# mountaindust/Parasitoids

Hardware: AMD Instinct MI355X
Metric: grid-days/sec on 4096^2 fp64 domain (higher is better)
Workload: dtype f64; 1 GPU; C3 synthetic stack: N=4097 (nominal 4096^2), 30 Gaussian day kernels K=2049, reference torus P=5121, FFT size 5184 (fast mode), prob model, one replica stack per GPU; dom_len=4097, ndays=30, P=5121, fft_len=5184, kernels_direct=False, full_column_pipeline=True

## Files before the change

parasitoids_amd/csrc/fft_colfull_kernels.h:

```cpp
#pragma once
#include "fft_rs_kernels.h"

struct ColFullArgs {
  const cplx* src;
  int64_t src_bstride;
  cplx* state;
  int64_t state_bstride;
  cplx* dst;
  int64_t dst_bstride;
  int ld, ncols, mode, store_prod;
  int nd;
  int dst_t;
  int dst_jb, dst_cc, dst_rst;
  int64_t src_dstride, dst_dstride;
  RowLive live;
  const unsigned long long* pred;
  double* pad_energy;
  int pad_row0, ncols_total;
  int col0;
  const cplx* alt_src;
  const unsigned long long* alt_pred;
  RowLive alt_live;
  FftProg prog;
};
// ... 263 lines not shown
#pragma unroll
          for (int q = 0; q < R1; ++q) x[q] = sst[jv + q * S::T1];
        }
        if (day + 1 < nd) fetch(day + 1, jv);
      }
      if constexpr (MODE == 0 && !CHAIN) {
        __syncthreads();
        if (jv < S::T3) {
#pragma unroll
          for (int q = 0; q < R3; ++q) ex[jv + q * S::T3] = x[q].x;
        }
        __syncthreads();
        if (jv < S::T1) {
#pragma unroll
          for (int q = 0; q < R1; ++q) x[q].x = ex[jv + q * S::T1];
        }
        __syncthreads();
        if (jv < S::T3) {
#pragma unroll
          for (int q = 0; q < R3; ++q) ex[jv + q * S::T3] = x[q].y;
        }
        __syncthreads();
        if (jv < S::T1) {
#pragma unroll
          for (int q = 0; q < R1; ++q) x[q].y = ex[jv + q * S::T1];
        }
        __syncthreads();
      }
      if constexpr (MODE == 0) {
        if (CHAIN) asm volatile("" : "+v"(w2.x), "+v"(w2.y), "+v"(w3.x), "+v"(w3.y));
        if (jv < S::T1) bfly<R1, PS_INV>(x);
        rs_tail<S, R1, R2, R3, PS_INV>(x, ex, jv, w2, w3);
        if (jv < S::T3) {
          const int64_t rst = a.dst_rst;
          const unsigned off = PS_COLFULL_OFF(a, c, jv);
          cplx* d = a.dst + (int64_t)blockIdx.y * a.dst_bstride + (int64_t)day * a.dst_dstride;
#pragma unroll
          for (int q = 0; q < R3; ++q) (d + (int64_t)(q * S::T3) * rst)[off] = x[q];
        }
        if (day + 1 < nd) __syncthreads();
      }
    }
    if (chain && a.store_prod && j < S::T3) {
#pragma unroll
      for (int q = 0; q < R3; ++q) st[j + q * S::T3] = sst[j + q * S::T3];
    }
  }
}


static __global__ void k_prefix_cols(cplx* state, cplx* khat, int L, int ncols, int nd) {
  const int k = blockIdx.x * blockDim.x + threadIdx.x;
  if (k >= L) return;
  const int64_t col = (int64_t)blockIdx.y * L + k;
  cplx p = state[col];
  for (int d = 0; d < nd; ++d) {
    cplx* e = khat + ((int64_t)d * ncols) * L + col;
    p = cmul(p, *e);
    *e = p;
  }
  state[col] = p;
}

template <int R1, int R2, int R3>
struct RsDual {
  using S = Rs<R1, R2, R3>;
  static constexpr int L = S::L;
  static constexpr int QA2 = (R2 + 1) / 2, QA3 = (R3 + 1) / 2;
  static constexpr int IA = QA2 * S::T2, IB = QA3 * S::T3;
  static constexpr int JA1 = IA / 16, JA2 = 16 * QA3;
  static constexpr int OFF1 = IA + IA / 16, OFF2 = IB + IB / 16;
  static constexpr int mx(int a, int b) { return a > b ? a : b; }
  static constexpr int MAXEL = mx(mx(IA, L - IA), mx(IB, L - IB));
  static constexpr int XH = (MAXEL + MAXEL / 16 + 32 + 15) & ~15;
  static constexpr size_t fixed_bytes = 2 * (size_t)XH * sizeof(double) + (size_t)L * sizeof(cplx);
  static constexpr long spare = (long)160 * 1024 - (long)fixed_bytes;
  static constexpr int CAP = spare > 0 ? (int)(spare / (64 * (long)sizeof(cplx))) * 64 : 0;
  static constexpr bool ok = S::NTHR <= 384 && CAP >= 512 &&
                             (S::RMAX <= 18 || (S::RMAX == 20 && (R2 * R3 == 20 * 14 || R2 * R3 == 20 * 16)));
  static constexpr size_t bytes = fixed_bytes + (size_t)CAP * sizeof(cplx);
  static_assert(S::T2 % 16 == 0 && S::T3 % 16 == 0, "half-pass offsets assume whole padding groups");
};

template <int R1, int R2, int R3>
__global__ void __launch_bounds__((2 * Rs<R1, R2, R3>::NTHR)) k_colfull_dual(ColFullArgs a) {
  using S = Rs<R1, R2, R3>;
  using D = RsDual<R1, R2, R3>;
  constexpr int L = S::L;
  constexpr int NW = S::NTHR / 64;
  if (pred_skip(a.pred)) return;
  const int b = blockIdx.x, xcd = b & 7, qq = b >> 3;
  const int c = a.col0 + ((((qq >> 3) << 3) + xcd) << 3) + (qq & 7);
  if (c >= a.ncols) return;
  const int role = threadIdx.x / S::NTHR;
  const int j0 = threadIdx.x - role * S::NTHR;
  double* exh = reinterpret_cast<double*>(ps_lds_raw) + role * D::XH;
  cplx* sst = reinterpret_cast<cplx*>(reinterpret_cast<double*>(ps_lds_raw) + 2 * D::XH);
  cplx* stage = sst + L;
  const FftProg& P = a.prog;
  const cplx w2c = tw_lookup(P.tw_lo, P.tw_hi, P.tw_shift, S::tw2(j0));
  const cplx w3c = tw_lookup(P.tw_lo, P.tw_hi, P.tw_shift, j0 < S::T3 ? S::tw3(j0) : 0);
  cplx* st = a.state + (int64_t)blockIdx.y * a.state_bstride + (int64_t)c * L;
  const int nd = a.nd;
  const int lane = j0 & 63, wave = j0 >> 6;

  auto live_of = [&](int day, int& a1, int& b1, int& a2, int& b2) {
    if (!a.live.on) { a1 = 0; b1 = L; a2 = L; b2 = L; return; }
    int lo = 0, hi = 0x3fffffff;
    if (a.live.range) { lo = a.live.range[2 * ((int)blockIdx.y + day)]; hi = a.live.range[2 * ((int)blockIdx.y + day) + 1]; }
    const SrcMap& m = a.live.map;
    a1 = max(0, lo - m.off1); b1 = min(m.n1, hi - m.off1 + 1);
    a2 = m.lo2 + max(0, lo - m.off2); b2 = min(L, m.lo2 + hi - m.off2 + 1);
    if (b1 < a1) b1 = a1;
    if (b2 < a2) b2 = a2;
    if (a2 < b1) a2 = b1;
  };
  auto stage_column = [&](int day) {
    int a1, b1, a2, b2;
    live_of(day, a1, b1, a2, b2);
    const int len1 = b1 - a1, tot = min(len1 + (b2 - a2), D::CAP);
    const cplx* sc = a.src + (int64_t)blockIdx.y * a.src_bstride + (int64_t)day * a.src_dstride + (int64_t)c * L;
    for (int ch = wave; ch * 64 < tot; ch += NW) {
      int e = ch * 64 + lane;
      e = e < tot ? e : tot - 1;
      const int n = e < len1 ? a1 + e : a2 + (e - len1);
      __builtin_amdgcn_global_load_lds(sc + n, (ps_lds_ptr)(stage + ch * 64), 16, 0, 0);
    }
  };

  if (role == 1) {
    stage_column(0);
    PS_WAIT_VM0();
  }
  PS_BAR_LDS();

  for (int slot = 0; slot <= nd; ++slot) {
    const bool act = role == 0 ? slot >= 1 : slot < nd;
    cplx x[S::RMAX];
    int j = j0;
    cplx w2 = w2c, w3 = w3c;
    asm volatile("" : "+v"(j), "+v"(w2.x), "+v"(w2.y), "+v"(w3.x), "+v"(w3.y));
    if (role == 0 && slot == 0) {
#pragma unroll 7
      for (int k = j; k < L; k += S::NTHR) sst[k] = st[k];
    }
    if (act && j < S::T1) {
      if (role == 0) {
#pragma unroll
        for (int q = 0; q < R1; ++q) x[q] = cconj(sst[j + q * S::T1]);
      } else {
        int a1, b1, a2, b2;
        live_of(slot, a1, b1, a2, b2);
        const int len1 = b1 - a1, len2 = b2 - a2;
        if (len1 + len2 <= D::CAP) {
#pragma unroll
          for (int q = 0; q < R1; ++q) {
            const int n = j + q * S::T1;
            const unsigned d1 = (unsigned)(n - a1), d2 = (unsigned)(n - a2);
            const bool in1 = d1 < (unsigned)len1, in2 = d2 < (unsigned)len2;
            const cplx v = stage[in1 ? d1 : (in2 ? len1 + d2 : 0u)];
            x[q] = (in1 || in2) ? v : make_double2(0.0, 0.0);
          }
        } else {
          const cplx* sc = a.src + (int64_t)blockIdx.y * a.src_bstride + (int64_t)slot * a.src_dstride + (int64_t)c * L;
#pragma unroll
          for (int q = 0; q < R1; ++q) {
            const int n = j + q * S::T1;
            x[q] = make_double2(0.0, 0.0);
            int e = -1;
            if (n >= a1 && n < b1) e = n - a1;
            else if (n >= a2 && n < b2) e = len1 + (n - a2);
            if (e >= 0) x[q] = e < D::CAP ? stage[e] : sc[n];
          }
        }
      }
      bfly<R1, PS_FWD>(x);
    }
#pragma unroll
    for (int part = 0; part < 2; ++part) {
      double keep[D::QA2];
#pragma unroll
      for (int h = 0; h < 2; ++h) {
        if (act && j < S::T1 && (j < D::JA1) == (h == 0)) {
          if (part) rs_put<R1, 1>(exh, S::x1_w(j) - h * D::OFF1, 1, x);
          else rs_put<R1, 0>(exh, S::x1_w(j) - h * D::OFF1, 1, x);
        }
        PS_BAR_LDS();
        if (part == 0 && h == 0 && role == 1 && slot + 1 < nd) stage_column(slot + 1);
        if (act && j < S::T2) {
          if (h == 0) {
#pragma unroll
            for (int q = 0; q < D::QA2; ++q) keep[q] = exh[S::x_r(j) + q * S::X1_RS];
          } else {
#pragma unroll
            for (int q = D::QA2; q < R2; ++q) {
              const double v = exh[S::x_r(j) + q * S::X1_RS - D::OFF1];
              if (part) x[q].y = v;
              else x[q].x = v;
            }
#pragma unroll
            for (int q = 0; q < D::QA2; ++q) {
              if (part) x[q].y = keep[q];
              else x[q].x = keep[q];
            }
          }
        }
        if (!(part == 1 && h == 1)) PS_BAR_LDS();
      }
    }
    asm volatile("" : "+v"(w2.x), "+v"(w2.y));
    if (act && j < S::T2) rs_stage<R2, PS_FWD>(x, w2, true);
    PS_BAR_LDS();
#pragma unroll
    for (int part = 0; part < 2; ++part) {
      double keep[D::QA3];
#pragma unroll
      for (int h = 0; h < 2; ++h) {
        if (act && j < S::T2 && (j < D::JA2) == (h == 0)) {
          if (part) rs_put<R2, 1>(exh, S::x2_w(j) - h * D::OFF2, 17, x);
          else rs_put<R2, 0>(exh, S::x2_w(j) - h * D::OFF2, 17, x);
        }
        PS_BAR_LDS();
        if (act && j < S::T3) {
          if (h == 0) {
#pragma unroll
            for (int q = 0; q < D::QA3; ++q) keep[q] = exh[S::x_r(j) + q * S::X2_RS];
          } else {
#pragma unroll
            for (int q = D::QA3; q < R3; ++q) {
              const double v = exh[S::x_r(j) + q * S::X2_RS - D::OFF2];
              if (part) x[q].y = v;
              else x[q].x = v;
            }
#pragma unroll
            for (int q = 0; q < D::QA3; ++q) {
              if (part) x[q].y = keep[q];
              else x[q].x = keep[q];
            }
          }
        }
        if (!(part == 1 && h == 1)) PS_BAR_LDS();
      }
    }
    asm volatile("" : "+v"(w3.x), "+v"(w3.y));
    if (act && j < S::T3) rs_stage<R3, PS_FWD>(x, w3, true);
    if (act && j < S::T3) {
      if (role == 0) {
        const int64_t rst = a.dst_rst;
        cplx* d = a.dst + (int64_t)blockIdx.y * a.dst_bstride + (int64_t)(slot - 1) * a.dst_dstride + PS_COLFULL_OFF(a, c, j);
#pragma unroll
        for (int q = 0; q < R3; ++q) d[(int64_t)(q * S::T3) * rst] = cconj(x[q]);
      } else {
#pragma unroll
        for (int q = 0; q < R3; ++q) {
          const cplx p = cmul(sst[j + q * S::T3], x[q]);
          sst[j + q * S::T3] = p;
        }
      }
    }
    if (role == 1 && slot == nd && a.store_prod) {
      for (int k = j; k < L; k += S::NTHR) st[k] = sst[k];
    }
    if (role == 0 && a.pad_energy) {
      double pe = 0.0;
      if (act && j < S::T3) {
        const int qlo = a.pad_row0 / S::T3;
#pragma unroll
        for (int q = 0; q < R3; ++q) {
          if (q < qlo) continue;
          if (q > qlo || j + q * S::T3 >= a.pad_row0) pe += x[q].x * x[q].x + x[q].y * x[q].y;
        }
      }
      pe = ps_wave_sum(pe);
      if (lane == 63) exh[D::XH - 8 + wave] = pe;
    }
    if (role == 1) PS_WAIT_VM0();
    PS_BAR_LDS();
    if (role == 0 && a.pad_energy && slot >= 1 && j0 == 0) {
      double e = 0.0;
      for (int w = 0; w < NW; ++w) e += exh[D::XH - 8 + w];
      a.pad_energy[((int64_t)blockIdx.y + (slot - 1)) * a.ncols_total + c] = e;
    }
  }
}
```

parasitoids_amd/csrc/ps_coldual.hip:

```cpp
#include "fft_colfull_kernels.h"
#include "rs_cfg.h"
#include "rs_launch.h"

template <int A, int B>
struct DualCfg {
  using D = RsDual<16, A, B>;
  using C = RsCfg<A, B>;
  static constexpr bool on = D::ok && C::CHAIN && C::LDSC > (size_t)80 * 1024;
};

bool rs_dual_ok(int r2, int r3) {
#define X(A, B) \
  if (r2 == A && r3 == B) return DualCfg<A, B>::on;
  PS_RS_SIZES(X)
#undef X
  return false;
}

int rs_coldual_set_attrs() {
#define X(A, B)                                                                                         \
  if constexpr (DualCfg<A, B>::on) {                                                                    \
    using DD = RsDual<16, A, B>;                                                                        \
    auto kern = k_colfull_dual<16, A, B>;                                                               \
    if (hipFuncSetAttribute((const void*)kern, hipFuncAttributeMaxDynamicSharedMemorySize, (int)DD::bytes) != hipSuccess) \
      return -1;                                                                                        \
  }
  PS_RS_SIZES(X)
#undef X
  return 0;
}

int rs_launch_coldual(int r2, int r3, const ColFullArgs& a, int lines8, int batch, hipStream_t st) {
  const dim3 grid((unsigned)(lines8 * 64), batch);
#define X(A, B)                                                                                         \
  if (r2 == A && r3 == B) {                                                                             \
    if constexpr (DualCfg<A, B>::on) {                                                                  \
      using DD = RsDual<16, A, B>;                                                                      \
      auto kern = k_colfull_dual<16, A, B>;                                                             \
      hipLaunchKernelGGL(kern, grid, dim3(2 * DD::S::NTHR), DD::bytes, st, a);                          \
      return 1;                                                                                         \
    }                                                                                                   \
    return 0;                                                                                           \
  }
  PS_RS_SIZES(X)
#undef X
  return 0;
}
```

parasitoids_amd/csrc/ps_config.h:

```cpp
#pragma once
#include <cstdlib>
#include <cstring>

#define PS_OPTION_TABLE(X)                                                                          \
                                               \
  X("PS_NO_RS", no_rs, 0, FLAG, C)                                                                  \
  X("PS_NO_RS_FWD", no_rs_fwd, 0, FLAG, C)                                                          \
  X("PS_NO_BIG_RADIX", no_big_radix, 0, FLAG, C)                                                    \
  X("PS_NO_TPIPE", no_tpipe, 0, FLAG, C)                                                            \
  X("PS_NO_FOLD_TPIPE", no_fold_tpipe, 0, FLAG, C)                                                  \
  X("PS_COL_SINGLE_MAX", col_single_max, 1200, INT, C)                                              \
  X("PS_COL_L1", col_l1, 0, INT, C)                                                                 \
  X("PS_CHUNK_DAYS", chunk_days, 0, INT, C)                                                         \
  X("PS_FAST_SIZE", fast_size, 0, INT, C)                                                           \
  X("PS_RS_AREA", rs_area, 0.0, NUM, C)                                                             \
                                                                                 \
  X("PS_COL_WSH", col_wsh, -1, INT, R)                                                              \
  X("PS_COL_THREADS", col_threads, 256, INT, R)                                                     \
  X("PS_FUSED_WSH", fused_wsh, -1, INT, R)                                                          \
  X("PS_FUSED_THREADS", fused_threads, 0, INT, R)                                                   \
  X("PS_FUSED_G", fused_g, 2, INT, R)                                                               \
  X("PS_MULTI_WSH", multi_wsh, -1, INT, R)                                                          \
  X("PS_DUAL_WSH", dual_wsh, -1, INT, R)                                                            \
  X("PS_FUSED_DAYS", fused_days, 8, INT, R)                                                         \
  X("PS_DIRECT_DAYS", direct_days, 4, INT, R)                                                       \
  X("PS_DIRECT_MAX_TERMS", direct_max_terms, 8, INT, R)                                             \
  X("PS_TPIPE_DAYS", tpipe_days, 32, INT, R)                                                        \
  X("PS_DUAL_MIN_DAYS", dual_min_days, 6, INT, R)                                                   \
                                                   \
  X("PS_TINV", tinv, 0, INT, R)                                                                     \
  X("PS_RSP", rsp, -1, INT, R)                                                                      \
  X("PS_ROW2", row2, -1, INT, R)                                                                    \
  X("PS_TPIPE", tpipe, -1, INT, R)                                                                  \
  X("PS_NO_PAIR_ROWS", no_pair_rows, 0, FLAG, R)                                                    \
  X("PS_TPIPE_SPLIT", tpipe_split, 0, INT, R)                                                       \
  X("PS_NO_CONJ", no_conj, 0, FLAG, R)                                                              \
  X("PS_NO_DUAL", no_dual, 0, FLAG, R)                                                              \
  X("PS_NO_DIRECT", no_direct, 0, FLAG, R)                                                          \
  X("PS_NO_ROW_BATCH", no_row_batch, 0, FLAG, R)                                                    \
  X("PS_NO_PAD_QUIET", no_pad_quiet, 0, FLAG, R)                                                    \
  X("PS_NO_TAIL_SPLIT", no_tail_split, 0, FLAG, R)                                                  \
  X("PS_NO_FWD_PERSIST", no_fwd_persist, 0, FLAG, R)                                                \
  X("PS_NO_FWD_SOLO", no_fwd_solo, 0, FLAG, R)                                                      \
  X("PS_FWD_STAGE", fwd_stage, 0, FLAG, R)                                                          \
  X("PS_NO_DEFER_REFFT", no_defer_refft, 0, FLAG, R)                                                \
  X("PS_NO_FILTER_CACHE", no_filter_cache, 0, FLAG, R)                                              \
  X("PS_NO_FOLD_FUSE", no_fold_fuse, 0, FLAG, R)                                                    \
  X("PS_NO_FOLD_ALT", no_fold_alt, 0, FLAG, R)                                                      \
  X("PS_NO_FOLD_ROWS", no_fold_rows, 0, FLAG, R)                                                    \
                                                                                 \
  X("PS_NO_SPECULATION", no_speculation, 0, FLAG, R)                                                \
  X("PS_SPEC_DEPTH", spec_depth, 2, INT, R)                                                         \
  X("PS_NO_FLAG_HISTORY", no_flag_history, 0, FLAG, R)                                              \
  X("PS_NO_WINDOW_HINT", no_window_hint, 0, FLAG, R)                                                \
  X("PS_NO_DEFER_CHECK", no_defer_check, 0, FLAG, R)                                                \
  X("PS_FIRST_WINDOW", first_window, -1, INT, R)                                                    \
  X("PS_KT_SPLIT", kt_split, -1, INT, R)                                                            \
  X("PS_NO_LAZY_KT", no_lazy_kt, 0, FLAG, R)                                                        \
  X("PS_NO_WIDE", no_wide, 0, FLAG, R)                                                              \
  X("PS_NO_ROUTE_HISTORY", no_route_history, 0, FLAG, R)                                            \
  X("PS_WIDE_MIN_N", wide_min_n, 1500, INT, R)                                                      \
  X("PS_AUTO_WINDOW", auto_window, 4, INT, R)                                                       \
                                                                  \
  X("PS_PM_SEG", pm_seg, 8, INT, R)                                                                 \
  X("PS_PM_SYNC", pm_sync, 0, FLAG, R)                                                              \
  X("PS_PM_NO_UNROLL", pm_no_unroll, 0, FLAG, R)

struct ps_config {
#define PS_CFG_FIELD_FLAG int
#define PS_CFG_FIELD_INT int
#define PS_CFG_FIELD_NUM double
#define X(key, field, dflt, kind, when) PS_CFG_FIELD_##kind field = dflt;
  PS_OPTION_TABLE(X)
#undef X
};

inline void ps_config_from_env(ps_config* c) {
  *c = ps_config();
#define PS_CFG_ENV_FLAG(field) c->field = (e[0] == '\0' || std::strcmp(e, "0") != 0) ? 1 : 0
#define PS_CFG_ENV_INT(field) c->field = std::atoi(e)
#define PS_CFG_ENV_NUM(field) c->field = std::atof(e)
#define X(key, field, dflt, kind, when) \
  if (const char* e = std::getenv(key)) { PS_CFG_ENV_##kind(field); }
  PS_OPTION_TABLE(X)
#undef X
}

inline int ps_config_set(ps_config* c, const char* key, double value, bool live) {
  if (!key) return -1;
#define PS_CFG_SET_FLAG(field) c->field = value != 0.0 ? 1 : 0
#define PS_CFG_SET_INT(field) c->field = (int)value
#define PS_CFG_SET_NUM(field) c->field = value
#define PS_CFG_WHEN_C true
#define PS_CFG_WHEN_R false
#define X(k, field, dflt, kind, when)         \
  if (std::strcmp(key, k) == 0) {             \
    if (live && PS_CFG_WHEN_##when) return -2; \
    PS_CFG_SET_##kind(field);                 \
    return 0;                                 \
  }
  PS_OPTION_TABLE(X)
#undef X
  return -1;
}

inline int ps_config_get(const ps_config* c, const char* key, double* value) {
  if (!key || !value) return -1;
#define X(k, field, dflt, kind, when) \
  if (std::strcmp(key, k) == 0) {     \
    *value = (double)c->field;        \
    return 0;                         \
  }
  PS_OPTION_TABLE(X)
#undef X
  return -1;
}
```

parasitoids_amd/csrc/ps_solver.hip:

```cpp
#include <deque>

#include "chain_kernels.h"
#include "fft_kernels.h"
#include "fft_colfull_kernels.h"
#include "rs_launch.h"
#include "row_fwd_stage.h"
#include "ps_common.h"
#include "ps_config.h"

thread_local std::string ps_tls_error;

extern "C" const char* ps_last_error(void) { return ps_tls_error.c_str(); }
extern "C" int ps_version(void) { return 100; }
extern "C" int ps_row_live_units(int P, int M, int np, int nd, const int32_t* ranges, int32_t* day, int32_t* unit, int cap) {
  if (!ranges && nd > 0) return -1;
  if (cap > 0 && (!day || !unit)) return -1;
  return rs_row_live_units(P, M, np, nd, ranges, day, unit, cap);
}
extern "C" int ps_row_fwd_info(int fft_len, int* np, int* persistent) {
  int r2 = 0, r3 = 0, n = 0, p = 0;
  if (!rs_lookup(fft_len, &r2, &r3) || !rs_row_fwd_info(r2, r3, &n, &p)) return -1;
  if (np) *np = n;
  if (persistent) *persistent = p;
  return 0;
// ... 443 lines not shown
  RsInfo info;
  if (s->rs_r2 == 0 || !rs_info(s->rs_r2, s->rs_r3, &info) || !info.rsp || knob == 0) return false;
  return knob == 1 || (s->tpipe && s->Pf >= 1536);
}

static int inter_layout(const ps_solver* s) {
  if (!s->tpipe) return 0;
  if (s->tinv) return 1;
  return (s->mode != PS_MODE_FOLD && !s->cfg.no_pair_rows && s->Pf % 2 == 0) ? 2 : 0;
}

static int launch_row_inv(ps_solver* s, const cplx* src, double* rec, int stat_slot, int batch,
                          double negval, double stat_scale, bool full_field = false,
                          double* const* recs_multi = nullptr, const int* pad_quiet = nullptr) {
  RowInvArgs a;
  a.pad_quiet = pad_quiet;
  a.persistent = (row_inv_persistent(s) && !(s->tpipe && s->tinv && !full_field)) ? 1 : 0;
  if (a.persistent && (s->cfg.row2 > 0 || (s->cfg.row2 < 0 && s->Pf >= 4096))) a.persistent = 2;
  a.nrec = 0;
  for (int i = 0; i < PS_MAX_GROUP_DAYS; ++i) a.rec_multi[i] = nullptr;
  if (recs_multi) {
    if (!a.persistent || batch > PS_MAX_GROUP_DAYS) return ps_fail(PS_ERR_STATE, "row pass: a record table needs the persistent kernel and at most %d entries", PS_MAX_GROUP_DAYS);
    a.nrec = batch;
    for (int i = 0; i < batch; ++i) a.rec_multi[i] = recs_multi[i];
  }
  a.src = src; a.src_bstride = (int64_t)s->Pf * s->ld;
  a.H = s->H; a.ld = s->ld; a.P = s->Pf; a.N = s->N;
  a.tstride = (s->tpipe && s->tinv && !full_field) ? s->Pf : 0;
  a.pair_src = (!full_field && inter_layout(s) == 2) ? 1 : 0;
  a.prog = s->row_plan.prog;
  a.rp = row_pairs(a.prog);
  a.scale = 1.0 / ((double)s->Pf * (double)s->Pf);
  a.rec = rec; a.rec_bstride = (int64_t)s->N * s->N;
  a.negval = negval; a.stat_scale = stat_scale;
  a.rowsum = s->rowsum.p + (int64_t)stat_slot * s->N;
  a.rowcnt = s->rowcnt.p + (int64_t)stat_slot * s->N;
  a.padmax = s->padmax.p + stat_slot;
  a.pad_floor = s->pad_floor;
  a.stat_bstride = s->N;
  if (full_field) {
    a.N = s->Pf;
    a.rec_bstride = (int64_t)s->Pf * s->Pf;
    a.rowsum = s->fold_rowsum.p; a.rowcnt = s->fold_rowcnt.p; a.padmax = s->fold_padmax.p;
    a.stat_bstride = s->Pf;
  }
  const int npairs = (s->Pf + 1) / 2;
  dim3 grid((npairs + a.rp - 1) / a.rp, batch);
  const int thr = row_threads(a.prog.L, s->row_big);
  const size_t lds = ((size_t)a.rp * row_pitch(a.prog) + a.prog.n_lo + a.prog.n_hi + a.prog.n_gen) * sizeof(cplx) +
                     4 * (thr / 64) * sizeof(double);
  if (lds > (size_t)kMaxLds) return ps_fail(PS_ERR_UNSUPPORTED, "row pass needs %zu B LDS", lds);
  ProfScope prof(s, !recs_multi ? PS_PROF_ROW_INV : batch == 2 ? PS_PROF_ROW_INV2 : batch == 4 ? PS_PROF_ROW_INV4
                                : batch == 8 ? PS_PROF_ROW_INV8 : batch == 1 ? PS_PROF_ROW_INV : PS_PROF_ROW_INVN,
                 recs_multi ? batch : 1);
  if (s->rs_r2 != 0) {
    if (!rs_launch_row_inv(s->rs_r2, s->rs_r3, a, npairs, batch, s->stream))
      return ps_fail(PS_ERR_STATE, "no register-resident row kernel for 16 x %d x %d", s->rs_r2, s->rs_r3);
  } else if (s->row_plan.generic)
    hipLaunchKernelGGL((k_row_inv<true, false>), grid, dim3(thr), lds, s->stream, a);
  else if (s->row_big)
    hipLaunchKernelGGL((k_row_inv<false, true>), grid, dim3(thr), lds, s->stream, a);
  else
    hipLaunchKernelGGL((k_row_inv<false, false>), grid, dim3(thr), lds, s->stream, a);
  PS_HIP(hipGetLastError());
  return PS_OK;
}

static bool colfull_dual(const ps_solver* s, int nd) {
  const int dual_min = s->cfg.dual_min_days;
  return dual_min > 0 && nd >= dual_min && rs_dual_ok(s->rs_r2, s->rs_r3);
}

static SrcMap map_plain(int n, int P);
struct ColAlt { const cplx* src; const unsigned long long* pred; RowLive live; };

static int launch_colfull(ps_solver* s, int mode, const cplx* src, cplx* state, int store_prod, cplx* dst, int batch,
                          RowLive live, const unsigned long long* pred, int nd = 1, double* pad_energy = nullptr,
                          int col0 = 0, int ncols = -1, int64_t state_bstride = -1, bool timed = true,
                          const ColAlt* alt = nullptr) {
  ColFullArgs a;
  a.pad_energy = nullptr;
  a.alt_src = nullptr; a.alt_pred = nullptr; a.alt_live = RowLive{0, {0, 0, 0, 0}, nullptr};
  if (alt) {
    if (!(mode == 0 && nd == 1 && batch == 1 && !pred) || s->refft_pending)
      return ps_fail(PS_ERR_STATE, "full-column pass: an alternative state source needs a plain single-day pass");
    a.alt_src = alt->src; a.alt_pred = alt->pred; a.alt_live = alt->live;
  }
  if (s->refft_pending) {
    if (!(mode == 0 && nd == 1 && batch == 1 && !pred && state == s->Ahat.p))
      return ps_fail(PS_ERR_STATE, "full-column pass: a flagged day's re-transform is still pending");
    a.alt_src = s->Trow.p; a.alt_pred = s->refft_pending;
    a.alt_live = RowLive{1, map_plain(s->N, s->Pf), nullptr};
  }
  a.pad_row0 = 2 * ((s->N + 1) / 2);
  a.ncols_total = s->H;
  a.col0 = col0;
  const int64_t spec = (int64_t)s->Pf * s->ld;
  a.src = src; a.src_bstride = spec;
  a.state = state; a.state_bstride = state_bstride >= 0 ? state_bstride : spec;
  a.dst = dst; a.dst_bstride = spec;
  a.ld = s->ld; a.ncols = ncols >= 0 ? ncols : s->H; a.mode = mode; a.store_prod = store_prod;
  a.nd = nd; a.src_dstride = spec; a.dst_dstride = spec;
  colfull_set_layout(a, s->tinv ? 1 : inter_layout(s), s->Pf);
  a.live = live;
  a.pred = pred;
  a.prog = s->row_plan.prog;
  const int groups = (a.ncols - col0 + 7) / 8;
  const int lines8 = (groups + 7) / 8;
  if (mode == 2) a.pad_energy = pad_energy;
  const bool prof_was = s->prof_on;
  if (!timed) s->prof_on = false;
  ProfScope prof(s, pred ? PS_PROF_REFFT
                          : (mode == 1 ? PS_PROF_COL_FWD_A
                                       : (nd == 2 ? PS_PROF_COL_INV_A2 : nd == 4 ? PS_PROF_COL_INV_A4
                                          : nd == 8 ? PS_PROF_COL_INV_A8 : nd == 1 ? PS_PROF_COL_INV_A : PS_PROF_COL_INV_AN)),
                 nd);
  s->prof_on = prof_was;
  if (mode == 0 && !pred && store_prod && colfull_dual(s, nd)) {
    a.pad_energy = pad_energy;
    if (!rs_launch_coldual(s->rs_r2, s->rs_r3, a, lines8, batch, s->stream))
      return ps_fail(PS_ERR_STATE, "two-role full-column pass: size 16 x %d x %d is not served", s->rs_r2, s->rs_r3);
    PS_HIP(hipGetLastError());
    return PS_OK;
  }
  if (!rs_launch_colfull(s->rs_r2, s->rs_r3, a, lines8, batch, s->stream))
    return ps_fail(PS_ERR_UNSUPPORTED, "full-column pass: size 16 x %d x %d cannot run this (chained days need the state column in LDS)",
                   s->rs_r2, s->rs_r3);
  PS_HIP(hipGetLastError());
  return PS_OK;
}

static bool colfull_chains(const ps_solver* s) {
  RsInfo info;
  return rs_info(s->rs_r2, s->rs_r3, &info) && info.chain;
}

static int fwd2d(ps_solver* s, const double* src, int64_t src_bstride, int src_ld, SrcMap rmap,
                 SrcMap cmap, cplx* out, int batch, const unsigned long long* pred, const int* rowrange = nullptr) {
  PS_TRY(launch_row_fwd(s, src, src_bstride, src_ld, rmap, cmap, s->T1.p, batch, pred, 1, rowrange));
  if (s->tpipe) return launch_colfull(s, 1, s->T1.p, out, 0, nullptr, batch, RowLive{1, rmap, rowrange}, pred);
  if (s->fwd_passes.size() == 1) {
    PS_TRY(launch_col<PS_FWD>(s, s->fwd_passes[0], s->T1.p, nullptr, nullptr, out, batch, 0, pred, RowLive{1, rmap, rowrange}));
  } else {
    PS_TRY(launch_col<PS_FWD>(s, s->fwd_passes[0], s->T1.p, nullptr, nullptr, s->T2.p, batch, 0, pred, RowLive{1, rmap, rowrange}));
    PS_TRY(launch_col<PS_FWD>(s, s->fwd_passes[1], s->T2.p, nullptr, nullptr, out, batch, 0, pred));
  }
  return PS_OK;
}

static int inv2d(ps_solver* s, const cplx* A, const cplx* B, cplx* prod, double* rec,
                 int stat_slot, double negval, double stat_scale) {
  if (s->tpipe) {
    if (B || prod) return ps_fail(PS_ERR_STATE, "inv2d: product form is not used by the full-column pipeline");
    PS_TRY(launch_colfull(s, 2, nullptr, const_cast<cplx*>(A), 0, s->T1.p, 1, RowLive{0, {0, 0, 0, 0}, nullptr}, nullptr));
    return launch_row_inv(s, s->T1.p, rec, stat_slot, 1, negval, stat_scale);
  }
  if (s->inv_passes.size() == 1) {
    PS_TRY(launch_col<PS_INV>(s, s->inv_passes[0], A, B, prod, s->T1.p, 1, 0, nullptr));
    PS_TRY(launch_row_inv(s, s->T1.p, rec, stat_slot, 1, negval, stat_scale));
  } else {
    PS_TRY(launch_col<PS_INV>(s, s->inv_passes[0], A, B, prod, s->T1.p, 1, 0, nullptr));
    PS_TRY(launch_col<PS_INV>(s, s->inv_passes[1], s->T1.p, nullptr, nullptr, s->T2.p, 1, 0, nullptr));
    PS_TRY(launch_row_inv(s, s->T2.p, rec, stat_slot, 1, negval, stat_scale));
  }
  return PS_OK;
}

static int fwd2d_partial(ps_solver* s, const double* src, int64_t src_bstride, int src_ld,
// ... 97 lines not shown
  ProfScope prof(s, nd == 1 ? PS_PROF_COL_INV_A : nd == 2 ? PS_PROF_COL_INV_A2 : nd == 4 ? PS_PROF_COL_INV_A4 : PS_PROF_COL_INV_A8);
  const int fenv = s->cfg.fused_threads;
  const int fthr = fenv > 0 ? fenv : (G == 2 && nd > 1 ? 512 : col_threads(s));
#define PS_MULTI_LAUNCH(ND, GG)                                                                                          \
  if (plan->generic) hipLaunchKernelGGL((k_col_fused_multi<true, ND, GG>), grid, dim3(fthr), need(a.wsh), s->stream, a); \
  else hipLaunchKernelGGL((k_col_fused_multi<false, ND, GG>), grid, dim3(fthr), need(a.wsh), s->stream, a)
  if (G == 2) {
    if (nd == 1) { PS_MULTI_LAUNCH(1, 2); }
    else if (nd == 2) { PS_MULTI_LAUNCH(2, 2); }
    else if (nd == 4) { PS_MULTI_LAUNCH(4, 2); }
    else { PS_MULTI_LAUNCH(8, 2); }
  } else {
    if (nd == 1) { PS_MULTI_LAUNCH(1, 1); }
    else if (nd == 2) { PS_MULTI_LAUNCH(2, 1); }
    else if (nd == 4) { PS_MULTI_LAUNCH(4, 1); }
    else { PS_MULTI_LAUNCH(8, 1); }
  }
#undef PS_MULTI_LAUNCH
  PS_HIP(hipGetLastError());
  *done = 1;
  return PS_OK;
}

static int launch_col_fused_dual(ps_solver* s, const cplx* kt, const cplx* state_part, RowLive state_live,
                                 cplx* dst, const int* rowrange, int* done) {
  ColFusedArgs a;
  DevPlan* plan = s->split ? &s->col_plan2 : &s->col_plan1;
  a.src = kt; a.state = const_cast<cplx*>(state_part); a.dst = dst;
  a.src_bstride = 0;
  a.ld = s->ld; a.ncols = s->H;
  a.L1 = s->split ? s->L1 : 1;
  a.L2 = s->split ? s->L2 : s->Pf;
  a.store_prod = 0;
  a.live = s->kt_live;
  a.live.range = rowrange;
  a.live2 = state_live;
  a.prog = plan->prog;
  a.dst_dstride = 0;
  fused_direct_args(s, a);
  a.wsh = std::min(col_wsh(s, a.prog.L), 4);
  if (s->cfg.dual_wsh >= 0) a.wsh = s->cfg.dual_wsh;
  auto need = [&](int wsh) {
    return (((size_t)a.prog.L << (wsh + 1)) + a.prog.n_lo + a.prog.n_hi + a.prog.n_gen) * sizeof(cplx);
  };
  while (need(a.wsh) > (size_t)kMaxLds && a.wsh > 2) --a.wsh;
  *done = 0;
  if (need(a.wsh) > (size_t)kMaxLds || s->cfg.no_dual) return PS_OK;
  const int W = 1 << a.wsh;
  const int ntiles = (s->H + W - 1) / W;
  dim3 grid((unsigned)((a.direct ? (ntiles + 7) / 8 * 8 : ntiles) * a.L1), 1);
  ProfScope prof(s, PS_PROF_COL_INV_A);
  const int fthr = s->cfg.fused_threads > 0 ? s->cfg.fused_threads : col_threads(s);
  if (plan->generic)
    hipLaunchKernelGGL(k_col_fused_dual<true>, grid, dim3(fthr), need(a.wsh), s->stream, a);
  else
    hipLaunchKernelGGL(k_col_fused_dual<false>, grid, dim3(fthr), need(a.wsh), s->stream, a);
  PS_HIP(hipGetLastError());
  *done = 1;
  return PS_OK;
}

static int conv_inv(ps_solver* s, const cplx* kt, cplx* state, int store_prod, double* rec,
                    int stat_slot, double negval, double stat_scale, const int* rowrange = nullptr) {
  if (s->tpipe) {
    RowLive live = s->kt_live;
    live.range = rowrange;
    const int split2 = s->cfg.tpipe_split;
    if (split2 && store_prod) {
      PS_TRY(launch_colfull(s, 3, kt, state, 1, nullptr, 1, live, nullptr));
      PS_TRY(launch_colfull(s, 2, nullptr, state, 0, s->T1.p, 1, RowLive{0, {0, 0, 0, 0}, nullptr}, nullptr));
    } else {
      PS_TRY(launch_colfull(s, 0, kt, state, store_prod, s->T1.p, 1, live, nullptr));
    }
    return launch_row_inv(s, s->T1.p, rec, stat_slot, 1, negval, stat_scale);
  }
  int done = 0;
  if (s->kt_direct && store_prod) PS_TRY(launch_col_fused_multi(s, kt, 1, state, s->T1.p, rowrange, &done));
  if (!done) PS_TRY(launch_col_fused(s, kt, state, store_prod, s->T1.p, rowrange));
  if (!s->split) return launch_row_inv(s, s->T1.p, rec, stat_slot, 1, negval, stat_scale);
  PS_TRY(launch_col<PS_INV>(s, s->inv_passes[1], s->T1.p, nullptr, nullptr, s->T2.p, 1, 0, nullptr));
  return launch_row_inv(s, s->T2.p, rec, stat_slot, 1, negval, stat_scale);
}

static int conv_inv_multi(ps_solver* s, const cplx* kt, int nd, cplx* state, double* const* recs, int d0,
                          double negval, double stat_scale, const int* rowrange, int* done) {
  const size_t spec = (size_t)s->Pf * s->ld;
  PS_TRY(s->T1.ensure(spec * nd));
  if (s->tpipe) {
    *done = 0;
    if (!colfull_chains(s)) return PS_OK;
    RowLive live = s->kt_live;
    live.range = rowrange;
    const bool batched_rows = row_inv_persistent(s) && !s->tinv && nd <= PS_MAX_GROUP_DAYS && !s->cfg.no_row_batch;
    const bool quiet = batched_rows && colfull_dual(s, nd) && s->N + 1 < s->Pf && !s->cfg.no_pad_quiet;
    if (quiet) {
      PS_TRY(s->pad_energy.ensure((size_t)nd * s->H));
      PS_TRY(s->pad_quiet.ensure(PS_MAX_GROUP_DAYS));
    }
    int hmain = s->H;
    if (!s->ncu) {
      int v = 0;
      if (hipDeviceGetAttribute(&v, hipDeviceAttributeMultiprocessorCount, s->device) == hipSuccess) s->ncu = v;
    }
    if (colfull_dual(s, nd) && s->ncu > 0 && s->H > s->ncu && !s->tinv && !s->cfg.no_tail_split) {
      const int rem = s->H % s->ncu;
      if (rem > 0 && rem * 3 <= s->ncu) hmain = s->H - rem;
    }
    PS_TRY(launch_colfull(s, 0, kt, state, 1, s->T1.p, 1, live, nullptr, nd, quiet ? s->pad_energy.p : nullptr, 0, hmain));
    if (hmain < s->H) {
      const int rem = s->H - hmain;
      PS_TRY(s->tail_hat.ensure((size_t)nd * rem * s->Pf));
      cplx* th = s->tail_hat.p - (int64_t)hmain * s->Pf;
      {
        ProfScope prof(s, PS_PROF_COL_TAIL, nd);
        PS_TRY(launch_colfull(s, 1, kt, th, 0, nullptr, nd, live, nullptr, 1, nullptr, hmain, s->H, (int64_t)rem * s->Pf, false));
        hipLaunchKernelGGL(k_prefix_cols, dim3((s->Pf + 255) / 256, rem), dim3(256), 0, s->stream,
                           state + (int64_t)hmain * s->Pf, s->tail_hat.p, s->Pf, rem, nd);
        PS_HIP(hipGetLastError());
        PS_TRY(launch_colfull(s, 2, nullptr, th, 0, s->T1.p, nd, RowLive{0, {0, 0, 0, 0}, nullptr}, nullptr, 1,
                              quiet ? s->pad_energy.p : nullptr, hmain, s->H, (int64_t)rem * s->Pf, false));
      }
    }
    if (quiet) {
      hipLaunchKernelGGL(k_pad_quiet, dim3(nd), dim3(256), 0, s->stream, s->pad_energy.p, s->H, (double)s->Pf,
                         1.0 / ((double)s->Pf * (double)s->Pf), s->pad_floor, s->pad_quiet.p);
      PS_HIP(hipGetLastError());
    }
    if (batched_rows) {
      PS_TRY(launch_row_inv(s, s->T1.p, nullptr, d0, nd, negval, stat_scale, false, recs, quiet ? s->pad_quiet.p : nullptr));
    } else {
      for (int i = 0; i < nd; ++i)
        PS_TRY(launch_row_inv(s, s->T1.p + i * spec, recs[i], d0 + i, 1, negval, stat_scale));
    }
    *done = 1;
    return PS_OK;
  }
  PS_TRY(launch_col_fused_multi(s, kt, nd, state, s->T1.p, rowrange, done));
  if (!*done) return PS_OK;
  for (int i = 0; i < nd; ++i) {
    cplx* t = s->T1.p + i * spec;
    if (s->split) {
      PS_TRY(launch_col<PS_INV>(s, s->inv_passes[1], t, nullptr, nullptr, s->T2.p, 1, 0, nullptr));
      t = s->T2.p;
    }
    PS_TRY(launch_row_inv(s, t, recs[i], d0 + i, 1, negval, stat_scale));
  }
  return PS_OK;
}

static SrcMap map_plain(int n, int P) { return SrcMap{n, 0, P, 0}; }
static SrcMap map_wrap(int m, int P) { return SrcMap{m + 1, m, P - m, 0}; }

static int ensure_record(ps_solver* s, int kind, int idx) {
  auto& v = s->recs[kind];
  if ((int)v.size() <= idx) v.resize(idx + 1, nullptr);
  if (!v[idx]) {
    hipError_t e = ps_dev_malloc((void**)&v[idx], (size_t)s->N * s->N * sizeof(double));
    if (e != hipSuccess) return ps_fail(PS_ERR_OOM, "record allocation failed: %s", hipGetErrorString(e));
  }
  return PS_OK;
}

static int ensure_stats(ps_solver* s, int n) {
  if (n <= s->nstat) return PS_OK;
  PS_TRY(s->rowsum.ensure((size_t)(n + 1) * s->N));
  PS_TRY(s->rowcnt.ensure((size_t)(n + 1) * s->N));
  PS_TRY(s->padmax.ensure(n + 1));
  PS_TRY(s->dstats.ensure(n + 1));
  s->nstat = n;
  return PS_OK;
}

static int finalize_days(ps_solver* s, int slot, int count, int renorm) {
  if (count <= 0) return PS_OK;
  hipLaunchKernelGGL(k_day_finalize, dim3(count), dim3(256), 0, s->stream,
                     s->rowsum.p + (int64_t)slot * s->N, s->rowcnt.p + (int64_t)slot * s->N,
                     s->padmax.p + slot, s->N, renorm, s->dstats.p + slot);
  PS_HIP(hipGetLastError());
  return PS_OK;
}

static int refft_if_flag(ps_solver* s, const double* rec, cplx* hat, int slot) {
  return fwd2d(s, rec, 0, s->N, map_plain(s->N, s->Pf), map_plain(s->N, s->Pf), hat, 1,
               s->padmax.p + slot);
}

static int refft_rows_if_flag(ps_solver* s, const double* rec, int slot) {
  PS_TRY(s->Trow.ensure((size_t)s->Pf * s->ld));
  const SrcMap m = map_plain(s->N, s->Pf);
  PS_TRY(launch_row_fwd(s, rec, 0, s->N, m, m, s->Trow.p, 1, s->padmax.p + slot, 1, nullptr));
  s->refft_pending = s->padmax.p + slot;
  return PS_OK;
}
static int resolve_refft(ps_solver* s) {
  if (!s->refft_pending) return PS_OK;
  const unsigned long long* pred = s->refft_pending;
  s->refft_pending = nullptr;
// ... 951 lines not shown
                             s->torus.p, s->recs[PS_REC_CHAIN][d], negval, stat_scale,
                             s->rowsum.p + (int64_t)d * s->N, s->rowcnt.p + (int64_t)d * s->N, s->padmax.p + d);
          PS_HIP(hipGetLastError());
          hipLaunchKernelGGL(k_truncate_if_flag, dim3(s->Pref), dim3(256), 0, s->stream, s->torus.p, s->Pref, s->N,
                             s->padmax.p + d);
          PS_HIP(hipGetLastError());
          continue;
        }
        PS_TRY(launch_row_fwd(s, s->torus.p, 0, s->Pref, tmap, tmap, s->T1.p, 1, nullptr, 1));
        const cplx* part = s->T1.p;
        cplx* fused_out = s->T2.p;
        RowLive part_live{1, tmap, nullptr};
        if (s->split) {
          PS_TRY(launch_col<PS_FWD>(s, s->fwd_passes[0], s->T1.p, nullptr, nullptr, s->T2.p, 1, 0, nullptr, part_live));
          part = s->T2.p;
          fused_out = s->T1.p;
          part_live = RowLive{0, {0, 0, 0, 0}, nullptr};
        }
        int dual = 0;
        PS_TRY(launch_col_fused_dual(s, B, part, part_live, fused_out, s->krange.p + 2 * d, &dual));
        if (!dual) {
          const ColPass& last = s->fwd_passes.back();
          PS_TRY(launch_col<PS_FWD>(s, last, part, nullptr, nullptr, s->Ahat.p, 1, 0, nullptr, part_live));
          PS_TRY(launch_col_fused(s, B, s->Ahat.p, 0, fused_out, s->krange.p + 2 * d));
        }
        if (s->split) {
          PS_TRY(launch_col<PS_INV>(s, s->inv_passes[1], s->T1.p, nullptr, nullptr, s->T2.p, 1, 0, nullptr));
          PS_TRY(launch_row_inv(s, s->T2.p, s->lin.p, d, 1, negval, stat_scale, true));
        } else {
          PS_TRY(launch_row_inv(s, s->T2.p, s->lin.p, d, 1, negval, stat_scale, true));
        }
        hipLaunchKernelGGL(k_fold, dim3(s->Pref), dim3(256), 0, s->stream, s->lin.p, s->Pf, s->Pref, s->N, s->M,
                           s->torus.p, s->recs[PS_REC_CHAIN][d], negval, stat_scale,
                           s->rowsum.p + (int64_t)d * s->N, s->rowcnt.p + (int64_t)d * s->N, s->padmax.p + d);
        PS_HIP(hipGetLastError());
        hipLaunchKernelGGL(k_truncate_if_flag, dim3(s->Pref), dim3(256), 0, s->stream, s->torus.p, s->Pref, s->N,
                           s->padmax.p + d);
        PS_HIP(hipGetLastError());
      }
    }
    return PS_OK;
  }
  s->spec_window = 2;
  if (s->cfg.no_speculation) s->speculate = false;
  const int hint = s->noflag_hint;
  s->noflag_hint = 0;
  bool hinted = false;
  int flagged_at = -1;
  const double flag_thr = s->auto_exact ? kCleanEps : 1e-8;
  int hint_abs = -1;
  if (s->auto_exact) {
    s->speculate = true;
    s->auto_first = -1;
    ++s->auto_runs;
    if (count > 0 && s->auto_hint == 0 && s->auto_runs % 16 != 0)
      return auto_handover(s, first, first, first + count, negval, stat_scale, renorm,
                           s->auto_first_regime == 1 ? 1.0 : 0.0);
    if (s->auto_hint > 0) hint_abs = first + s->auto_hint;
  }
  std::vector<char> hist;
  if (!s->auto_exact && !s->speculate && s->hist_count == count && s->hist_first == first && count >= 2 &&
      !s->cfg.no_flag_history && !s->cfg.no_speculation) {
    PS_HIP(hipEventSynchronize(s->hist_ev));
    hist.resize(count);
    for (int i = 0; i < count; ++i) {
      double m;
      __builtin_memcpy(&m, &s->hhist[i], sizeof(double));
      hist[i] = !(m <= 1e-8);
    }
  }
  s->hist_count = 0;
  if (s->speculate || !hist.empty()) {
    for (int i = 0; i < 2; ++i)
      if (!s->spec_ev[i]) PS_HIP(hipEventCreateWithFlags(&s->spec_ev[i], hipEventDisableTiming));
    if (s->hflags_n < first + count) {
      if (s->hflags) (void)hipHostFree(s->hflags);
      s->hflags = nullptr;
      s->hflags_n = 0;
      PS_HIP(hipHostMalloc((void**)&s->hflags, (size_t)(first + count) * sizeof(unsigned long long), hipHostMallocDefault));
      s->hflags_n = first + count;
    }
  }
  if (s->tpipe_ok && !s->spec_valid) set_pipeline(s, want_full_column(s, first, count));
  PS_TRY(ensure_spectrum(s));
  if (s->speculate && s->tpipe && colfull_chains(s) && hint >= count && count >= 4 && !s->cfg.no_window_hint) {
    int w0 = s->cfg.first_window > 0 ? s->cfg.first_window : count;
    w0 = std::max(2, std::min(std::min(w0, count), PS_MAX_GROUP_DAYS));
    s->spec_window = w0;
    hinted = true;
  }
  bool guided = false;
  if (!hist.empty() && s->tpipe && colfull_chains(s))
    for (int i = 0; i + 1 < count && !guided; ++i) guided = !hist[i] && !hist[i + 1];
  const bool defer_ok = !s->cfg.no_defer_check && s->mode == PS_MODE_FAST && !s->auto_exact && !s->borrowed &&
                        s->tpipe && s->speculate && !guided && count <= s->chunk_days;
  for (int c0 = first; c0 < first + count; c0 += s->chunk_days) {
    const int cn = std::min(s->chunk_days, first + count - c0);
    const int split_days = s->cfg.kt_split >= 0 ? s->cfg.kt_split : (hinted ? s->spec_window : 14);
    const bool lazy_tail = s->auto_exact && hint_abs >= c0 && hint_abs + 2 < c0 + cn &&
                           !s->cfg.no_lazy_kt;
    if (s->kt_early) {
      s->kt_early = false;
    } else if (!lazy_tail && s->tpipe && s->speculate && split_days > 0 && cn >= split_days + (hinted ? 4 : 8)) {
      if (!s->stream2) {
        int lo = 0, hi = 0;
        (void)hipDeviceGetStreamPriorityRange(&lo, &hi);
        PS_HIP(hipStreamCreateWithPriority(&s->stream2, hipStreamNonBlocking, lo));
        PS_HIP(hipEventCreateWithFlags(&s->kt_ev, hipEventDisableTiming));
        PS_HIP(hipEventCreateWithFlags(&s->kt_ev0, hipEventDisableTiming));
      }
      PS_TRY(transform_kernels(s, c0, split_days, 0, cn));
      PS_HIP(hipEventRecord(s->kt_ev0, s->stream));
      PS_HIP(hipStreamWaitEvent(s->stream2, s->kt_ev0, 0));
      hipStream_t main_stream = s->stream;
      s->stream = s->stream2;
      const int rc2 = transform_kernels(s, c0 + split_days, cn - split_days, split_days, cn);
      s->stream = main_stream;
      if (rc2 != PS_OK) return rc2;
      PS_HIP(hipEventRecord(s->kt_ev, s->stream2));
      s->kt_from = c0 + split_days;
    } else if (lazy_tail) {
      const int now = hint_abs + 2 - c0;
      bool direct_all = direct_possible(s);
      for (int q = c0; q < c0 + cn && direct_all; ++q) direct_all = day_is_compact(s, q);
      s->kt_lazy_direct = direct_all ? 1 : 0;
      PS_TRY(transform_kernels(s, c0, now, 0, cn, s->kt_lazy_direct));
      s->kt_lazy_from = c0 + now;
      s->kt_lazy_c0 = c0;
      s->kt_lazy_cn = cn;
    } else {
      PS_TRY(transform_kernels(s, c0, cn));
    }
    auto day = [&](int d, bool with_refft) -> int { return run_day(s, d, with_refft, negval, stat_scale); };
    struct Win { int d0, w, ev; };
    std::deque<Win> q;
    (void)flagged_at;
    int d = c0, nev = 0;
    while (true) {
      if (!s->speculate && !guided) {
        for (; d < c0 + cn; ++d) PS_TRY(day(d, true));
        break;
      }
      const size_t depth = (size_t)std::max(1, s->cfg.spec_depth);
      while (q.size() < depth && d < c0 + cn && !(hint_abs >= 0 && d == hint_abs + 1 && !q.empty())) {
        int w = std::min(s->spec_window, c0 + cn - d);
        if (hint_abs >= d) w = std::min(w, hint_abs - d + 1);
        if (guided) {
          int g = 0;
          while (d + g < c0 + cn && g < PS_MAX_GROUP_DAYS && !hist[d + g - first]) ++g;
          if (g < 2) {
            PS_TRY(day(d, true));
            ++d;
            continue;
          }
          w = g;
          PS_TRY(resolve_refft(s));
        }
        for (int i = 0; i < w;) {
          int g = 0;
          const int direct_days = s->cfg.direct_days;
          const int tpipe_days = std::min(PS_MAX_GROUP_DAYS, std::max(1, s->cfg.tpipe_days));
          const int maxd = s->tpipe ? std::min(s->fused_days >= 8 ? PS_MAX_GROUP_DAYS : s->fused_days, tpipe_days)
                                    : (s->kt_direct ? std::min(s->fused_days, direct_days) : s->fused_days);
          if (maxd > 1 && w - i >= 2) {
            int nd = s->tpipe ? std::min(maxd, w - i)
                              : (maxd >= 8 && w - i >= 8) ? 8 : (maxd >= 4 && w - i >= 4) ? 4 : 2;
            while (nd > 2 && s->T1.ensure((size_t)s->Pf * s->ld * nd) == PS_ERR_OOM) {
              (void)hipGetLastError();
              nd = std::max(2, nd / 2);
              s->cfg.tpipe_days = std::min(s->cfg.tpipe_days, nd);
            }
            PS_TRY(kernels_ready(s, d + i + nd - 1));
            const cplx* B = s->Bhat.p + (size_t)(d + i - s->bhat_first) * s->Pf * s->ld;
            PS_TRY(conv_inv_multi(s, B, nd, s->Ahat.p, &s->recs[PS_REC_CHAIN][d + i], d + i, negval, stat_scale,
                                  s->krange.p + 2 * (d + i), &g));
            if (g) g = nd;
            else s->fused_days = 1;
          }
          if (!g) {
            PS_TRY(day(d + i, false));
            g = 1;
          }
          i += g;
        }
        PS_HIP(hipMemcpyAsync(s->hflags + d, s->padmax.p + d, (size_t)w * sizeof(unsigned long long),
                              hipMemcpyDeviceToHost, s->stream));
        PS_HIP(hipEventRecord(s->spec_ev[nev & 1], s->stream));
        q.push_back(Win{d, w, nev & 1});
        ++nev;
        d += w;
        s->spec_window = hinted ? PS_MAX_GROUP_DAYS : std::min(64, 2 * s->spec_window);
      }
      if (q.empty()) break;
      const Win x = q.front();
      if (defer_ok && q.size() == 1 && d >= c0 + cn) {
        s->pend.on = true;
        s->pend.first = first; s->pend.count = count;
        s->pend.d0 = x.d0; s->pend.w = x.w; s->pend.ev = x.ev;
        s->pend.negval = negval; s->pend.stat_scale = stat_scale;
        s->pend.thr = flag_thr;
        ++s->n_deferred;
        return PS_OK;
      }
      q.pop_front();
      PS_HIP(hipEventSynchronize(s->spec_ev[x.ev]));
      const int f = first_flagged_day(s, x.d0, x.w, flag_thr);
      if (f < 0) continue;
      q.clear();
      flagged_at = f;
      if (s->auto_exact) {
        double mf;
        __builtin_memcpy(&mf, &s->hflags[f], sizeof(double));
        return auto_handover(s, first, f, first + count, negval, stat_scale, renorm, mf);
      }
      guided = false;
      PS_TRY(recover_from_flag(s, f, d));
// ... 721 lines not shown
```

parasitoids_amd/csrc/rs_launch.h:

```cpp
#pragma once
#include <hip/hip_runtime.h>
#include "fft_kernels.h"

struct ColFullArgs;

struct RsInfo {
  int np, nthr;
  size_t lds_rows, lds_col1, lds_colc;
  bool chain;
  bool rsp;
};
bool rs_lookup(int L, int* r2, int* r3);
int rs_next_size(int n);
bool rs_info(int r2, int r3, RsInfo* out);
int rs_rows_set_attrs();
int rs_colfull_set_attrs();
int rs_launch_row_fwd(int r2, int r3, const RowFwdArgs& a, int npairs, int batch, hipStream_t st);
int rs_launch_row_inv(int r2, int r3, const RowInvArgs& a, int npairs, int batch, hipStream_t st);
bool rs_row_fwd_info(int r2, int r3, int* np, int* persistent);
int rs_launch_row_fwd_live(int r2, int r3, const RowFwdArgs& a, const int* hranges, int batch, hipStream_t st,
                           bool stage, bool solo);
size_t rs_row_fwd_stage_lds(int r2, int r3, int src_ld);
bool rs_row_fwd_staged(int r2, int r3, int src_ld);
int rs_row_live_units(int P, int M, int np, int nd, const int* ranges, int* day, int* unit, int cap);
int rs_launch_colfull(int r2, int r3, const ColFullArgs& a, int lines8, int batch, hipStream_t st);
struct RowFoldArgs;
int rs_launch_row_fold(int r2, int r3, const RowFoldArgs& a, int units, hipStream_t st);
bool rs_colfull_alt_ok(int r2, int r3);
bool rs_dual_ok(int r2, int r3);
int rs_coldual_set_attrs();
int rs_launch_coldual(int r2, int r3, const ColFullArgs& a, int lines8, int batch, hipStream_t st);
```

Baseline: 4452 grid-days/s.

## Fuse initial state column FFT into the first dual-role column window pass

Measured after the change: 4526 grid-days/s, median of 6. 1.7% higher.

```diff
diff --git a/parasitoids_amd/csrc/fft_colfull_kernels.h b/parasitoids_amd/csrc/fft_colfull_kernels.h
--- a/parasitoids_amd/csrc/fft_colfull_kernels.h
+++ b/parasitoids_amd/csrc/fft_colfull_kernels.h
@@ -369,7 +369,7 @@
   static_assert(S::T2 % 16 == 0 && S::T3 % 16 == 0, "half-pass offsets assume whole padding groups");
 };
 
-template <int R1, int R2, int R3>
+template <int R1, int R2, int R3, bool SF = false>
 __global__ void __launch_bounds__((2 * Rs<R1, R2, R3>::NTHR)) k_colfull_dual(ColFullArgs a) {
   using S = Rs<R1, R2, R3>;
   using D = RsDual<R1, R2, R3>;
@@ -422,17 +422,25 @@
   PS_BAR_LDS();
 
   for (int slot = 0; slot <= nd; ++slot) {
-    const bool act = role == 0 ? slot >= 1 : slot < nd;
+    const bool act = role == 0 ? (SF || slot >= 1) : slot < nd;
     cplx x[S::RMAX];
     int j = j0;
     cplx w2 = w2c, w3 = w3c;
     asm volatile("" : "+v"(j), "+v"(w2.x), "+v"(w2.y), "+v"(w3.x), "+v"(w3.y));
-    if (role == 0 && slot == 0) {
+    if (!SF && role == 0 && slot == 0) {
 #pragma unroll 7
       for (int k = j; k < L; k += S::NTHR) sst[k] = st[k];
     }
     if (act && j < S::T1) {
-      if (role == 0) {
+      if (SF && role == 0 && slot == 0) {
+        const cplx* ss = a.alt_src + (int64_t)c * L;
+#pragma unroll
+        for (int q = 0; q < R1; ++q) {
+          const int n = j + q * S::T1;
+          x[q] = make_double2(0.0, 0.0);
+          if (row_live(a.alt_live, n, 0)) x[q] = ss[n];
+        }
+      } else if (role == 0) {
 #pragma unroll
         for (int q = 0; q < R1; ++q) x[q] = cconj(sst[j + q * S::T1]);
       } else {
@@ -531,7 +539,14 @@
     }
     asm volatile("" : "+v"(w3.x), "+v"(w3.y));
     if (act && j < S::T3) rs_stage<R3, PS_FWD>(x, w3, true);
-    if (act && j < S::T3) {
+    if (SF && slot == 0) {
+      if (role == 0 && j < S::T3) {
+#pragma unroll
+        for (int q = 0; q < R3; ++q) sst[j + q * S::T3] = x[q];
+      }
+      PS_BAR_LDS();
+    }
+    if (act && j < S::T3 && !(SF && slot == 0 && role == 0)) {
       if (role == 0) {
         const int64_t rst = a.dst_rst;
         cplx* d = a.dst + (int64_t)blockIdx.y * a.dst_bstride + (int64_t)(slot - 1) * a.dst_dstride + PS_COLFULL_OFF(a, c, j);
@@ -550,7 +565,7 @@
     }
     if (role == 0 && a.pad_energy) {
       double pe = 0.0;
-      if (act && j < S::T3) {
+      if (act && j < S::T3 && !(SF && slot == 0)) {
         const int qlo = a.pad_row0 / S::T3;
 #pragma unroll
         for (int q = 0; q < R3; ++q) {
diff --git a/parasitoids_amd/csrc/ps_coldual.hip b/parasitoids_amd/csrc/ps_coldual.hip
--- a/parasitoids_amd/csrc/ps_coldual.hip
+++ b/parasitoids_amd/csrc/ps_coldual.hip
@@ -7,6 +7,7 @@
   using D = RsDual<16, A, B>;
   using C = RsCfg<A, B>;
   static constexpr bool on = D::ok && C::CHAIN && C::LDSC > (size_t)80 * 1024;
+  static constexpr bool sf = on && D::S::RMAX <= 18;
 };
 
 bool rs_dual_ok(int r2, int r3) {
@@ -17,13 +18,28 @@
   return false;
 }
 
+bool rs_dual_state_ok(int r2, int r3) {
+#define X(A, B) \
+  if (r2 == A && r3 == B) return DualCfg<A, B>::sf;
+  PS_RS_SIZES(X)
+#undef X
+  return false;
+}
+
+static int dual_set_attr(const void* kern, size_t bytes) {
+  return hipFuncSetAttribute(kern, hipFuncAttributeMaxDynamicSharedMemorySize, (int)bytes) == hipSuccess ? 0 : -1;
+}
+
 int rs_coldual_set_attrs() {
 #define X(A, B)                                                                                         \
   if constexpr (DualCfg<A, B>::on) {                                                                    \
     using DD = RsDual<16, A, B>;                                                                        \
     auto kern = k_colfull_dual<16, A, B>;                                                               \
-    if (hipFuncSetAttribute((const void*)kern, hipFuncAttributeMaxDynamicSharedMemorySize, (int)DD::bytes) != hipSuccess) \
-      return -1;                                                                                        \
+    if (dual_set_attr((const void*)kern, DD::bytes) != 0) return -1;                                    \
+    if constexpr (DualCfg<A, B>::sf) {                                                                  \
+      auto kern_sf = k_colfull_dual<16, A, B, true>;                                                    \
+      if (dual_set_attr((const void*)kern_sf, DD::bytes) != 0) return -1;                               \
+    }                                                                                                   \
   }
   PS_RS_SIZES(X)
 #undef X
@@ -36,6 +52,15 @@
   if (r2 == A && r3 == B) {                                                                             \
     if constexpr (DualCfg<A, B>::on) {                                                                  \
       using DD = RsDual<16, A, B>;                                                                      \
+      if (a.alt_src) {                                                                                  \
+        if constexpr (DualCfg<A, B>::sf) {                                                              \
+          if (batch != 1 || a.pred) return 0;                                                           \
+          auto kern_sf = k_colfull_dual<16, A, B, true>;                                                \
+          hipLaunchKernelGGL(kern_sf, grid, dim3(2 * DD::S::NTHR), DD::bytes, st, a);                   \
+          return 1;                                                                                     \
+        }                                                                                               \
+        return 0;                                                                                       \
+      }                                                                                                 \
       auto kern = k_colfull_dual<16, A, B>;                                                             \
       hipLaunchKernelGGL(kern, grid, dim3(2 * DD::S::NTHR), DD::bytes, st, a);                          \
       return 1;                                                                                         \
diff --git a/parasitoids_amd/csrc/ps_config.h b/parasitoids_amd/csrc/ps_config.h
--- a/parasitoids_amd/csrc/ps_config.h
+++ b/parasitoids_amd/csrc/ps_config.h
@@ -40,6 +40,7 @@
   X("PS_NO_ROW_BATCH", no_row_batch, 0, FLAG, R)                                                    \
   X("PS_NO_PAD_QUIET", no_pad_quiet, 0, FLAG, R)                                                    \
   X("PS_NO_TAIL_SPLIT", no_tail_split, 0, FLAG, R)                                                  \
+  X("PS_NO_STATE_FUSE", no_state_fuse, 0, FLAG, R)                                                  \
   X("PS_NO_FWD_PERSIST", no_fwd_persist, 0, FLAG, R)                                                \
   X("PS_NO_FWD_SOLO", no_fwd_solo, 0, FLAG, R)                                                      \
   X("PS_FWD_STAGE", fwd_stage, 0, FLAG, R)                                                          \
diff --git a/parasitoids_amd/csrc/ps_solver.hip b/parasitoids_amd/csrc/ps_solver.hip
--- a/parasitoids_amd/csrc/ps_solver.hip
+++ b/parasitoids_amd/csrc/ps_solver.hip
@@ -549,8 +549,10 @@
   a.pad_energy = nullptr;
   a.alt_src = nullptr; a.alt_pred = nullptr; a.alt_live = RowLive{0, {0, 0, 0, 0}, nullptr};
   if (alt) {
-    if (!(mode == 0 && nd == 1 && batch == 1 && !pred) || s->refft_pending)
-      return ps_fail(PS_ERR_STATE, "full-column pass: an alternative state source needs a plain single-day pass");
+    const bool fused_window = nd > 1 && store_prod && colfull_dual(s, nd) && rs_dual_state_ok(s->rs_r2, s->rs_r3);
+    if (!(mode == 0 && (nd == 1 || fused_window) && batch == 1 && !pred) || s->refft_pending)
+      return ps_fail(PS_ERR_STATE, "full-column pass: an alternative state source needs a plain single-day pass "
+                                   "or a two-role window");
     a.alt_src = alt->src; a.alt_pred = alt->pred; a.alt_live = alt->live;
   }
   if (s->refft_pending) {
@@ -814,10 +816,19 @@
   return launch_row_inv(s, s->T2.p, rec, stat_slot, 1, negval, stat_scale);
 }
 
+static int ensure_spectrum(ps_solver* s);
+static bool state_fuse_ok(const ps_solver* s, int nd) {
+  return s->tpipe && s->mode == PS_MODE_FAST && !s->auto_exact && !s->borrowed && !s->refft_pending && !s->tinv &&
+         !s->cfg.no_state_fuse && colfull_dual(s, nd) && rs_dual_state_ok(s->rs_r2, s->rs_r3) &&
+         !s->recs[PS_REC_STATE].empty() && s->recs[PS_REC_STATE][0];
+}
+
 static int conv_inv_multi(ps_solver* s, const cplx* kt, int nd, cplx* state, double* const* recs, int d0,
                           double negval, double stat_scale, const int* rowrange, int* done) {
   const size_t spec = (size_t)s->Pf * s->ld;
   PS_TRY(s->T1.ensure(spec * nd));
+  const bool fuse_state = !s->spec_valid && state == s->Ahat.p && colfull_chains(s) && state_fuse_ok(s, nd);
+  if (!fuse_state) PS_TRY(ensure_spectrum(s));
   if (s->tpipe) {
     *done = 0;
     if (!colfull_chains(s)) return PS_OK;
@@ -838,13 +849,25 @@
       const int rem = s->H % s->ncu;
       if (rem > 0 && rem * 3 <= s->ncu) hmain = s->H - rem;
     }
-    PS_TRY(launch_colfull(s, 0, kt, state, 1, s->T1.p, 1, live, nullptr, nd, quiet ? s->pad_energy.p : nullptr, 0, hmain));
+    ColAlt salt{nullptr, nullptr, RowLive{0, {0, 0, 0, 0}, nullptr}};
+    if (fuse_state) {
+      PS_TRY(s->Trow.ensure(spec));
+      const SrcMap m = map_plain(s->N, s->Pf);
+      const int* srows = s->srange_valid ? s->srange.p : nullptr;
+      PS_TRY(launch_row_fwd(s, s->recs[PS_REC_STATE][0], 0, s->N, m, m, s->Trow.p, 1, nullptr, 1, srows));
+      salt = ColAlt{s->Trow.p, nullptr, RowLive{1, m, srows}};
+    }
+    PS_TRY(launch_colfull(s, 0, kt, state, 1, s->T1.p, 1, live, nullptr, nd, quiet ? s->pad_energy.p : nullptr, 0, hmain,
+                          -1, true, fuse_state ? &salt : nullptr));
+    if (fuse_state) s->spec_valid = true;
     if (hmain < s->H) {
       const int rem = s->H - hmain;
       PS_TRY(s->tail_hat.ensure((size_t)nd * rem * s->Pf));
       cplx* th = s->tail_hat.p - (int64_t)hmain * s->Pf;
       {
         ProfScope prof(s, PS_PROF_COL_TAIL, nd);
+        if (fuse_state)
+          PS_TRY(launch_colfull(s, 1, s->Trow.p, state, 0, nullptr, 1, salt.live, nullptr, 1, nullptr, hmain, s->H, -1, false));
         PS_TRY(launch_colfull(s, 1, kt, th, 0, nullptr, nd, live, nullptr, 1, nullptr, hmain, s->H, (int64_t)rem * s->Pf, false));
         hipLaunchKernelGGL(k_prefix_cols, dim3((s->Pf + 255) / 256, rem), dim3(256), 0, s->stream,
                            state + (int64_t)hmain * s->Pf, s->tail_hat.p, s->Pf, rem, nd);
@@ -1962,12 +1985,16 @@
     }
   }
   if (s->tpipe_ok && !s->spec_valid) set_pipeline(s, want_full_column(s, first, count));
-  PS_TRY(ensure_spectrum(s));
   if (s->speculate && s->tpipe && colfull_chains(s) && hint >= count && count >= 4 && !s->cfg.no_window_hint) {
     int w0 = s->cfg.first_window > 0 ? s->cfg.first_window : count;
     w0 = std::max(2, std::min(std::min(w0, count), PS_MAX_GROUP_DAYS));
     s->spec_window = w0;
     hinted = true;
+  }
+  {
+    const int w1 = std::min(std::min(s->spec_window, std::min(s->chunk_days, count)),
+                            std::min(PS_MAX_GROUP_DAYS, std::max(1, s->cfg.tpipe_days)));
+    if (!(hinted && !s->spec_valid && s->fused_days >= 8 && state_fuse_ok(s, w1))) PS_TRY(ensure_spectrum(s));
   }
   bool guided = false;
   if (!hist.empty() && s->tpipe && colfull_chains(s))
@@ -2011,7 +2038,10 @@
     } else {
       PS_TRY(transform_kernels(s, c0, cn));
     }
-    auto day = [&](int d, bool with_refft) -> int { return run_day(s, d, with_refft, negval, stat_scale); };
+    auto day = [&](int d, bool with_refft) -> int {
+      PS_TRY(ensure_spectrum(s));
+      return run_day(s, d, with_refft, negval, stat_scale);
+    };
     struct Win { int d0, w, ev; };
     std::deque<Win> q;
     (void)flagged_at;
diff --git a/parasitoids_amd/csrc/rs_launch.h b/parasitoids_amd/csrc/rs_launch.h
--- a/parasitoids_amd/csrc/rs_launch.h
+++ b/parasitoids_amd/csrc/rs_launch.h
@@ -28,5 +28,6 @@
 int rs_launch_row_fold(int r2, int r3, const RowFoldArgs& a, int units, hipStream_t st);
 bool rs_colfull_alt_ok(int r2, int r3);
 bool rs_dual_ok(int r2, int r3);
+bool rs_dual_state_ok(int r2, int r3);
 int rs_coldual_set_attrs();
 int rs_launch_coldual(int r2, int r3, const ColFullArgs& a, int lines8, int batch, hipStream_t st);
```
